# WeiZhang1988/YDORBSLAM

Hardware: AMD Instinct MI355X
Metric: ORB extract+match Mkeypoints/sec (higher is better)
Workload: dtype u8

## Files before the change

### ydorbslam_amd/csrc/extract_kernels.hip.h

```cpp
#pragma once
#include <hip/hip_runtime.h>
#include <stdint.h>

#include "quadtree_core.h"
#include "quadtree_flat.h"

#pragma clang fp contract(off)

namespace ydorb {

constexpr int kPad = 19;
constexpr int kBorder = 16;
constexpr int kMaxLevels = 8;
constexpr int kTileMax = 72;
#ifndef QT_THREADS
#define QT_THREADS 512
#endif
constexpr int kQtThreads = QT_THREADS;

struct LevelDev {
  int w, h, pitch;
  int padOff;
  int blurOff, blurPitch;
  int cellBegin, nCells;
  int quota;
  int candOff;
  int kpOff;
  int tabOff;
  int nodeTabOff;
  float scale;
  float size;
};
struct PlanDev {
  int nLevels, nCellsTotal, cellCap, sumQuota;
  int maxX[16];
  unsigned nodeTabFrameStride;
  int blurTileBegin[kMaxLevels + 1];
  int borderBegin[kMaxLevels + 1];
  LevelDev lv[kMaxLevels];
};
#ifndef BLUR_TH
#define BLUR_TH 58
#endif
constexpr int kBlurTW = 64, kBlurTH = BLUR_TH;
struct CellDev {
  short level, x0, y0, x1, y1, pad0;
  int srcOff;
};

__device__ __forceinline__ int reflect101(int i, int n) {
  if (n == 1) return 0;
  while (i < 0 || i >= n) i = i < 0 ? -i : 2 * (n - 1) - i;
  return i;
}

typedef uint32_t __attribute__((aligned(1))) u32_unaligned;
typedef unsigned long long __attribute__((aligned(1))) u64_unaligned;

#ifndef PYR_ROWS
#define PYR_ROWS 8
#endif
constexpr int kPyrRows = PYR_ROWS;
__global__ __launch_bounds__(256) void k_pyr_level0(const uint8_t* __restrict__ img, int stride, size_t frameStride,
                                                    uint8_t* __restrict__ pyr, size_t pyrFrameStride, LevelDev L) {
  const int wx = blockIdx.x * 64 + (threadIdx.x & 63);
  const int yb = (blockIdx.y * 4 + __builtin_amdgcn_readfirstlane(threadIdx.x >> 6)) * kPyrRows;
  const int x0 = wx * 4 - kPad;
  if (x0 + 3 < 0 || x0 >= L.w) return;
  const uint8_t* src = img + (size_t)blockIdx.z * frameStride;
  uint8_t* dst = pyr + (size_t)blockIdx.z * pyrFrameStride + L.padOff + (size_t)kPad * L.pitch + wx * 4;
  const int xa = L.w >= 4 ? min(max(x0, 0), L.w - 4) : 0, sh = 8 * (x0 - xa);
  uint32_t v[kPyrRows];
#pragma unroll
  for (int r = 0; r < kPyrRows; r++) {
    const uint8_t* row = src + (size_t)min(yb + r, L.h - 1) * stride;
    if (L.w >= 4) {
      v[r] = *reinterpret_cast<const u32_unaligned*>(row + xa);
    } else {
      v[r] = 0;
      for (int b = 0; b < L.w; b++) v[r] |= (uint32_t)row[b] << (8 * b);
    }
    v[r] = sh < 0 ? v[r] << (-sh) : v[r] >> sh;
  }
#pragma unroll
  for (int r = 0; r < kPyrRows; r++)
    if (yb + r < L.h) *reinterpret_cast<uint32_t*>(dst + (size_t)(yb + r) * L.pitch) = v[r];
}

__global__ __launch_bounds__(256) void k_pyr_resize(uint8_t* __restrict__ pyr, size_t pyrFrameStride, LevelDev Lp, LevelDev L,
                                                    double scaleX, const short* __restrict__ alpha,
                                                    const int* __restrict__ yofs, const short* __restrict__ beta) {
  const int wx = blockIdx.x * 64 + (threadIdx.x & 63);
  const int yb = (blockIdx.y * 4 + __builtin_amdgcn_readfirstlane(threadIdx.x >> 6)) * kPyrRows;
  const int x0 = wx * 4 - kPad;
  if (x0 + 3 < 0 || x0 >= L.w) return;
  uint8_t* frame = pyr + (size_t)blockIdx.z * pyrFrameStride;
  const uint8_t* S = frame + Lp.padOff + (size_t)kPad * Lp.pitch + kPad;
  uint8_t* dst = frame + L.padOff + (size_t)kPad * L.pitch + wx * 4;
  int sx[4], sx1[4], a0[4], a1[4];
#pragma unroll
  for (int b = 0; b < 4; b++) {
    const int dx = min(max(x0 + b, 0), L.w - 1);
    const float fx = (float)__dsub_rn(__dmul_rn((double)dx + 0.5, scaleX), 0.5);
    sx[b] = min(max((int)floorf(fx), 0), Lp.w - 1);
    a0[b] = alpha[2 * dx]; a1[b] = alpha[2 * dx + 1];
    sx1[b] = min(sx[b] + 1, Lp.w - 1);
  }
  const bool fast = sx[3] - sx[0] <= 6;
  const uint8_t *r0p[kPyrRows], *r1p[kPyrRows];
  int b0[kPyrRows], b1[kPyrRows];
#pragma unroll
  for (int r = 0; r < kPyrRows; r++) {
    const int dy = min(yb + r, L.h - 1);
    const int sy = yofs[dy];
    b0[r] = beta[2 * dy]; b1[r] = beta[2 * dy + 1];
    r0p[r] = S + (size_t)min(max(sy, 0), Lp.h - 1) * Lp.pitch;
    r1p[r] = S + (size_t)min(max(sy + 1, 0), Lp.h - 1) * Lp.pitch;
  }
  uint32_t v[kPyrRows];
  if (fast) {
    typedef unsigned short u16x2 __attribute__((ext_vector_type(2)));
    uint32_t sel[4];
    u16x2 ab[4];
#pragma unroll
    for (int b = 0; b < 4; b++) {
      const uint32_t off = (uint32_t)(sx[b] - sx[0]);
      sel[b] = off | 0x0c000c00u | ((off + 1) << 16);
      ab[b] = u16x2{(unsigned short)a0[b], (unsigned short)a1[b]};
    }
    unsigned long long w0[kPyrRows], w1[kPyrRows];
#pragma unroll
    for (int r = 0; r < kPyrRows; r++) {
      w0[r] = *reinterpret_cast<const u64_unaligned*>(r0p[r] + sx[0]);
      w1[r] = *reinterpret_cast<const u64_unaligned*>(r1p[r] + sx[0]);
    }
#pragma unroll
    for (int r = 0; r < kPyrRows; r++) {
      v[r] = 0;
#pragma unroll
      for (int b = 0; b < 4; b++) {
        const uint32_t p0 = __builtin_amdgcn_perm((uint32_t)(w0[r] >> 32), (uint32_t)w0[r], sel[b]);
        const uint32_t p1 = __builtin_amdgcn_perm((uint32_t)(w1[r] >> 32), (uint32_t)w1[r], sel[b]);
        const int h0 = (int)__builtin_amdgcn_udot2(__builtin_bit_cast(u16x2, p0), ab[b], 0u, false);
        const int h1 = (int)__builtin_amdgcn_udot2(__builtin_bit_cast(u16x2, p1), ab[b], 0u, false);
        const int o = (((b0[r] * (h0 >> 4)) >> 16) + ((b1[r] * (h1 >> 4)) >> 16) + 2) >> 2;
        v[r] |= (uint32_t)(o & 0xFF) << (8 * b);
      }
    }
  } else {
#pragma unroll
    for (int r = 0; r < kPyrRows; r++) {
      v[r] = 0;
#pragma unroll
      for (int b = 0; b < 4; b++) {
        const int h0 = r0p[r][sx[b]] * a0[b] + r0p[r][sx1[b]] * a1[b];
        const int h1 = r1p[r][sx[b]] * a0[b] + r1p[r][sx1[b]] * a1[b];
        const int o = (((b0[r] * (h0 >> 4)) >> 16) + ((b1[r] * (h1 >> 4)) >> 16) + 2) >> 2;
        v[r] |= (uint32_t)(o & 0xFF) << (8 * b);
      }
    }
  }
#pragma unroll
  for (int r = 0; r < kPyrRows; r++)
    if (yb + r < L.h) *reinterpret_cast<uint32_t*>(dst + (size_t)(yb + r) * L.pitch) = v[r];
}

struct PyrPadEntry { uint32_t laneA4, laneB4, selM, selF; };
struct PyrColEntry { uint32_t sel[4]; uint32_t ab[4]; };
constexpr uint32_t kPermIdentity = 0x03020100u;
#ifndef PYR_ROWS_F
#define PYR_ROWS_F 8
#endif
constexpr int kPyrRowsF = PYR_ROWS_F;

__device__ __forceinline__ uint32_t pyr_finish_dword(uint32_t v, const PyrPadEntry& pe) {
  const uint32_t A = (uint32_t)__builtin_amdgcn_ds_bpermute((int)pe.laneA4, (int)v);
  const uint32_t B = (uint32_t)__builtin_amdgcn_ds_bpermute((int)pe.laneB4, (int)v);
  const uint32_t M = __builtin_amdgcn_perm(A, B, pe.selM);
  return __builtin_amdgcn_perm(M, v, pe.selF);
}
__device__ __forceinline__ void pyr_store_rows(uint8_t* dst, int pitch, int y, int h, uint32_t v) {
  if (y >= h) return;
  *reinterpret_cast<uint32_t*>(dst + (ptrdiff_t)y * pitch) = v;
  if (y >= 1 && y <= kPad) *reinterpret_cast<uint32_t*>(dst - (ptrdiff_t)y * pitch) = v;
  if (y >= h - 1 - kPad && y <= h - 2) *reinterpret_cast<uint32_t*>(dst + (ptrdiff_t)(2 * (h - 1) - y) * pitch) = v;
}

__global__ __launch_bounds__(256) void k_pyr_level0_f(const uint8_t* __restrict__ img, int stride, size_t frameStride,
                                                      uint8_t* __restrict__ pyr, size_t pyrFrameStride, LevelDev L,
                                                      const PyrPadEntry* __restrict__ padTab, int shift) {
  const int wx = blockIdx.x * 64 + (threadIdx.x & 63) - shift;
  const int yb = (blockIdx.y * 4 + __builtin_amdgcn_readfirstlane(threadIdx.x >> 6)) * kPyrRowsF;
  const int nd = (L.w + 2 * kPad + 3) >> 2;
  if (wx < 0 || wx >= nd) return;
  const int x0 = wx * 4 - kPad;
  const uint8_t* src = img + (size_t)blockIdx.z * frameStride;
  uint8_t* dst = pyr + (size_t)blockIdx.z * pyrFrameStride + L.padOff + (size_t)kPad * L.pitch + wx * 4;
// ... 794 lines not shown
#pragma unroll
      for (int jj = 0; jj < 4; jj++) { key[jj] = (int)(st[4 * g + jj] & 0xFFFu); slot[jj] = qf_off(Pn) + (key[jj] >> (2 * (D - Pn))); }
      for (int d = Pn - 1; d >= 1; d--) {
        const int off = qf_off(d), sh = 2 * (D - d);
#pragma unroll
        for (int jj = 0; jj < 4; jj++) {
          const int sl = off + (key[jj] >> sh);
          if (hist[sl] == 1) slot[jj] = sl;
        }
      }
#pragma unroll
      for (int jj = 0; jj < 4; jj++) st[4 * g + jj] = (st[4 * g + jj] & 0xFFFF0000u) | (uint32_t)slot[jj];
    }
  }
  if (!pairs) {
    const int TQ = ((1 << (2 * Pn)) - 1) / 3;
    const int per = (TQ + NT - 1) / NT;
    constexpr int MAXQ = ((1 << (2 * D)) - 1) / 3 / NT + 1;
    uint2 qv[MAXQ];
    int qslot[MAXQ];
    unsigned flags = 0, cntF = 0;
#pragma unroll
    for (int t = 0; t < MAXQ; t++) {
      qslot[t] = -1; qv[t] = make_uint2(0, 0);
      const int q = tid * per + t;
      if (t < per && q < TQ) {
        int d = Pn, start = 0;
        while (q >= start + (1 << (2 * (d - 1)))) { start += 1 << (2 * (d - 1)); d--; }
        const int pq = q - start;
        const int bq = pq ^ (int)(qt_flat_mask(d) >> 2);
        qslot[t] = qf_off(d) + 4 * bq;
        qv[t] = *reinterpret_cast<const QT_LDS uint2*>(hist + qslot[t]);
        const unsigned c[4] = {qv[t].x & 0xFFFFu, qv[t].x >> 16, qv[t].y & 0xFFFFu, qv[t].y >> 16};
        const unsigned sum = c[0] + c[1] + c[2] + c[3];
#pragma unroll
        for (int e = 0; e < 4; e++) {
          const unsigned cn = c[3 - e];
          const bool fl = sum >= 2 && (d == Pn ? cn >= 1 : cn == 1);
          flags |= (unsigned)fl << (4 * t + e);
          cntF += fl;
        }
      }
    }
    unsigned total;
    unsigned pos = block_scan_excl(cntF, &total);
    if ((int)total != K) { give_up(); return; }
#pragma unroll
    for (int t = 0; t < MAXQ; t++) {
      if (qslot[t] >= 0) {
        const unsigned c[4] = {qv[t].x & 0xFFFFu, qv[t].x >> 16, qv[t].y & 0xFFFFu, qv[t].y >> 16};
        unsigned o[4];
#pragma unroll
        for (int e = 0; e < 4; e++) {
          const unsigned cn = c[3 - e];
          unsigned v = 0x7FFFu;
          if ((flags >> (4 * t + e)) & 1u) {
            if ((int)pos < nOut) {
              v = pos | (cn > 16 ? 0x8000u : 0u);
              if (cn > 16) nodeBig[pos] = 1;
            }
            pos++;
          }
          o[3 - e] = v;
        }
        *reinterpret_cast<QT_LDS uint2*>(hist + qslot[t]) = make_uint2(o[0] | (o[1] << 16), o[2] | (o[3] << 16));
      }
    }
  }
  __syncthreads();

#pragma unroll
  for (int g = 0; g < ITEMS / 4; g++) {
    if (4 * g * NT < n) {
      unsigned pv[4];
#pragma unroll
      for (int jj = 0; jj < 4; jj++) pv[jj] = pairs ? st[4 * g + jj] & 0x7FFFu : hist[st[4 * g + jj] & 0xFFFFu] & 0x7FFFu;
#pragma unroll
      for (int jj = 0; jj < 4; jj++) {
        const int i = (4 * g + jj) * NT + tid;
        const bool ok = i < n && (int)pv[jj] < nOut;
        const unsigned k = ok ? pv[jj] : (unsigned)(quotaMax + 1);
        const uint32_t rs = st[4 * g + jj] & 0xFFFF0000u;
        __hip_atomic_fetch_max(nodeLo + k, ok ? rs | (0xFFFFu - (uint32_t)i) : 0u, __ATOMIC_RELAXED, __HIP_MEMORY_SCOPE_WORKGROUP);
        __hip_atomic_fetch_max(nodeHi + k, ok ? rs | (uint32_t)i : 0u, __ATOMIC_RELAXED, __HIP_MEMORY_SCOPE_WORKGROUP);
        st[4 * g + jj] = rs | (ok ? k : 0xFFFFu);
      }
    }
  }
  __syncthreads();
  for (int k = tid; k < nOut; k += NT) {
    const unsigned iLo = 0xFFFFu - (nodeLo[k] & 0xFFFFu), iHi = nodeHi[k] & 0xFFFFu;
    if (iLo == iHi || !nodeBig[k]) {
      outKp[k] = fetch((int)iLo);
    } else {
      const int s = atomicAdd(&sTieN, 1);
      if (s < kQfMaxTied) { sTieNode[s] = k; nodeBig[k] = (uint8_t)(2 + s); }
    }
  }
  __syncthreads();
  const int nTied = sTieN;
  if (nTied > kQfMaxTied) { give_up(); return; }
  if (nTied > 0) {
    const int slotCap = kQfTieCap / nTied;
    QT_LDS uint32_t* tKey = (QT_LDS uint32_t*)smem;
    QT_LDS uint32_t* tVal = tKey + kQfTieCap;
#pragma unroll
    for (int j = 0; j < ITEMS; j++) {
      if (j * NT < n) {
        const unsigned k = st[j] & 0xFFFFu;
        if (k != 0xFFFFu) {
          const unsigned tb = nodeBig[k];
          if (tb >= 2) {
            const int s = (int)tb - 2, idx = atomicAdd(&sTieCnt[s], 1);
            if (idx < slotCap) { tKey[s * slotCap + idx] = (uint32_t)(j * NT + tid); tVal[s * slotCap + idx] = st[j] >> 16; }
            else sFlag = 1;
          }
        }
      }
    }
    __syncthreads();
    if (sFlag) { give_up(); return; }
    for (int s = 0; s < nTied; s++) {
      const int m = sTieCnt[s];
      constexpr int MAXM = (kQfTieCap + NT - 1) / NT;
      int rk[MAXM];
      uint32_t oi[MAXM], rr[MAXM];
#pragma unroll
      for (int t = 0; t < MAXM; t++) {
        rk[t] = -1; oi[t] = 0; rr[t] = 0;
        const int e = tid + NT * t;
        if (e < m) {
          oi[t] = tKey[s * slotCap + e];
          rr[t] = tVal[s * slotCap + e];
          int r = 0;
          for (int u = 0; u < m; u++) r += tKey[s * slotCap + u] < oi[t];
          rk[t] = r;
        }
      }
      __syncthreads();
#pragma unroll
      for (int t = 0; t < MAXM; t++)
        if (rk[t] >= 0) { tKey[s * slotCap + rk[t]] = (rr[t] << 16) | (uint32_t)rk[t]; tVal[s * slotCap + rk[t]] = oi[t]; }
      __syncthreads();
    }
    if (tid < nTied) {
      const int m = sTieCnt[tid];
      const int best = qt_sort_front(tKey + tid * slotCap, m);
      outKp[sTieNode[tid]] = fetch((int)tVal[tid * slotCap + best]);
    }
  }
  if (tid == 0) { needPass[unit] = 0; lvlCount[unit] = nOut; }
}

__global__ __launch_bounds__(256) void k_blur(const uint8_t* __restrict__ pyr, size_t pyrFrameStride, uint8_t* __restrict__ blur,
                                              size_t blurFrameStride, PlanDev P) {
  constexpr int TW = kBlurTW, TH = kBlurTH, SH = TH + 6, SWW = 18;
  __shared__ uint32_t src[SH * SWW];
  __shared__ __align__(16) uint32_t hb[(SH / 2) * TW];
  int f = blockIdx.y, tileId = blockIdx.x;
  if ((f | 7) < (int)gridDim.y) {
    tileId = (f & 7) * (gridDim.x >> 3) + (blockIdx.x >> 3);
    f = (f & ~7) | (blockIdx.x & 7);
  }
  if (tileId >= P.blurTileBegin[P.nLevels]) return;
  int level = 0;
#pragma unroll
  for (int l = 1; l < kMaxLevels; l++)
    if (l < P.nLevels && tileId >= P.blurTileBegin[l]) level = l;
  tileId -= P.blurTileBegin[level];
  const LevelDev L = P.lv[level];
  const int tilesX = (L.w + TW - 1) / TW;
  const int ty = tileId / tilesX, tx = tileId - ty * tilesX;
  const int x0 = tx * TW, y0 = ty * TH;
  const uint8_t* padded = pyr + (size_t)f * pyrFrameStride + L.padOff;
  {
    const int r0 = threadIdx.x / SWW, wd = threadIdx.x - r0 * SWW;
    const int pcol = x0 + 16 + 4 * wd;
    const bool colOk = pcol < L.pitch;
    if (r0 < 14)
#pragma unroll
      for (int r = r0; r < SH; r += 14) {
        const int prow = min(y0 + r + kPad - 3, L.h + 2 * kPad - 1);
        src[r * SWW + wd] = colOk ? *reinterpret_cast<const uint32_t*>(padded + (size_t)prow * L.pitch + pcol) : 0u;
      }
  }
  __syncthreads();
  for (int task = threadIdx.x; task < (SH / 2) * (TW / 4); task += 256) {
    const int rp = task >> 4, g = task & 15;
    uint32_t o[2][4];
#pragma unroll
    for (int h = 0; h < 2; h++) {
      const int r = 2 * rp + h;
      const uint32_t w0 = src[r * SWW + g], w1 = src[r * SWW + g + 1], w2 = src[r * SWW + g + 2];
#pragma unroll
      for (int k = 0; k < 4; k++) {
        const uint32_t lo4 = k ? __builtin_amdgcn_alignbyte(w1, w0, k) : w0, hi4 = k ? __builtin_amdgcn_alignbyte(w2, w1, k) : w1;
        o[h][k] = __builtin_amdgcn_udot4(hi4, 0x00122230u, __builtin_amdgcn_udot4(lo4, 0x38302212u, 0u, false), false);
      }
    }
    *reinterpret_cast<uint4*>(&hb[rp * TW + g * 4]) =
        make_uint4(o[0][0] | (o[1][0] << 16), o[0][1] | (o[1][1] << 16), o[0][2] | (o[1][2] << 16), o[0][3] | (o[1][3] << 16));
  }
  __syncthreads();
  const int c4 = (threadIdx.x & 15) * 4;
#pragma unroll
  for (int r = threadIdx.x >> 4; r < TH; r += 16) {
    const int gy = y0 + r;
    if (!(gy < L.h && x0 + c4 < L.blurPitch)) continue;
    typedef unsigned short u16x2 __attribute__((ext_vector_type(2)));
    const bool odd = r & 1;
    const u16x2 k0 = odd ? u16x2{0, 18} : u16x2{18, 34}, k1 = odd ? u16x2{34, 48} : u16x2{48, 56};
    const u16x2 k2 = odd ? u16x2{56, 48} : u16x2{48, 34}, k3 = odd ? u16x2{34, 18} : u16x2{18, 0};
    const uint32_t* hp = &hb[(r >> 1) * TW + c4];
    const uint4 p0 = *reinterpret_cast<const uint4*>(hp), p1 = *reinterpret_cast<const uint4*>(hp + TW);
    const uint4 p2 = *reinterpret_cast<const uint4*>(hp + 2 * TW), p3 = *reinterpret_cast<const uint4*>(hp + 3 * TW);
    const uint32_t q0[4] = {p0.x, p0.y, p0.z, p0.w}, q1[4] = {p1.x, p1.y, p1.z, p1.w}, q2[4] = {p2.x, p2.y, p2.z, p2.w}, q3[4] = {p3.x, p3.y, p3.z, p3.w};
    uint32_t acc[4];
#pragma unroll
    for (int k = 0; k < 4; k++) {
      acc[k] = __builtin_amdgcn_udot2(__builtin_bit_cast(u16x2, q0[k]), k0, 32768u, false);
      acc[k] = __builtin_amdgcn_udot2(__builtin_bit_cast(u16x2, q1[k]), k1, acc[k], false);
      acc[k] = __builtin_amdgcn_udot2(__builtin_bit_cast(u16x2, q2[k]), k2, acc[k], false);
      acc[k] = __builtin_amdgcn_udot2(__builtin_bit_cast(u16x2, q3[k]), k3, acc[k], false);
    }
    const uint32_t out = (acc[0] >> 16) | ((acc[1] >> 16) << 8) | ((acc[2] >> 16) << 16) | ((acc[3] >> 16) << 24);
    *reinterpret_cast<uint32_t*>(blur + (size_t)f * blurFrameStride + L.blurOff + (size_t)gy * L.blurPitch + x0 + c4) = out;
  }
}

__device__ __forceinline__ float fast_atan2_deg(float y, float x) {
  const float p1 = 0.9997878412794807f * (float)(180 / 3.14159265358979323846);
  const float p3 = -0.3258083974640975f * (float)(180 / 3.14159265358979323846);
  const float p5 = 0.1555786518463281f * (float)(180 / 3.14159265358979323846);
  const float p7 = -0.04432655554792128f * (float)(180 / 3.14159265358979323846);
  const float eps = (float)2.2204460492503131e-16;
  const float ax = fabsf(x), ay = fabsf(y);
  float a, c, c2;
  if (ax >= ay) {
    c = __fdiv_rn(ay, __fadd_rn(ax, eps));
    c2 = __fmul_rn(c, c);
    a = __fmul_rn(__fadd_rn(__fmul_rn(__fadd_rn(__fmul_rn(__fadd_rn(__fmul_rn(p7, c2), p5), c2), p3), c2), p1), c);
  } else {
    c = __fdiv_rn(ax, __fadd_rn(ay, eps));
    c2 = __fmul_rn(c, c);
    a = __fsub_rn(90.f, __fmul_rn(__fadd_rn(__fmul_rn(__fadd_rn(__fmul_rn(__fadd_rn(__fmul_rn(p7, c2), p5), c2), p3), c2), p1), c));
  }
  if (x < 0) a = __fsub_rn(180.f, a);
  if (y < 0) a = __fsub_rn(360.f, a);
  return a;
}

__device__ __forceinline__ void sincos_det(float xf, float* sinOut, float* cosOut) {
  const double x = (double)xf;
  const double n = rint(__dmul_rn(x, 6.36619772367581382433e-01));
  const double r = __dsub_rn(__dsub_rn(x, __dmul_rn(n, 1.57079632673412561417e+00)), __dmul_rn(n, 6.07710050650619224932e-11));
  const double z = __dmul_rn(r, r);
  double p = __dmul_rn(z, 1.58969099521155010221e-10);
  p = __dadd_rn(p, -2.50507602534068634195e-08); p = __dmul_rn(p, z);
  p = __dadd_rn(p, 2.75573137070700676789e-06);  p = __dmul_rn(p, z);
  p = __dadd_rn(p, -1.98412698298579493134e-04); p = __dmul_rn(p, z);
  p = __dadd_rn(p, 8.33333333332248946124e-03);  p = __dmul_rn(p, z);
  p = __dadd_rn(p, -1.66666666666666324348e-01); p = __dmul_rn(p, z);
  p = __dmul_rn(p, r); p = __dadd_rn(p, r);
  double q = __dmul_rn(z, -1.13596475577881948265e-11);
  q = __dadd_rn(q, 2.08757232129817482790e-09);  q = __dmul_rn(q, z);
  q = __dadd_rn(q, -2.75573143513906633035e-07); q = __dmul_rn(q, z);
  q = __dadd_rn(q, 2.48015872894767294178e-05);  q = __dmul_rn(q, z);
  q = __dadd_rn(q, -1.38888888888741095749e-03); q = __dmul_rn(q, z);
  q = __dadd_rn(q, 4.16666666666666019037e-02);  q = __dmul_rn(q, z);
  q = __dmul_rn(q, z);
  double h = __dmul_rn(z, 0.5);
  h = __dsub_rn(h, q);
  h = __dsub_rn(1.0, h);
  const int quad = ((int)n) & 3;
  const double sv = quad == 0 ? p : quad == 1 ? h : quad == 2 ? -p : -h;
  const double cv = quad == 0 ? h : quad == 1 ? -p : quad == 2 ? -h : p;
  *sinOut = (float)sv;
  *cosOut = (float)cv;
}

__device__ __align__(16) const float kPatternDev[1024] = {
#include "orb_pattern_data.inc"
};

struct YdKeyPointDev { float x, y, size, angle, response; int octave, class_id; };

__global__ __launch_bounds__(256) void k_orient_describe(const uint8_t* __restrict__ pyr, size_t pyrFrameStride,
                                                         const uint8_t* __restrict__ blur, size_t blurFrameStride, PlanDev P,
                                                         const uint32_t* __restrict__ lvlKp, const int* __restrict__ lvlCount,
                                                         YdKeyPointDev* __restrict__ kps, uint8_t* __restrict__ desc, int cap,
                                                         int* __restrict__ nOut, float* __restrict__ lvlAngle) {
  const int lane = threadIdx.x & 63;
  int bx = blockIdx.x, f = blockIdx.y;
  if ((f | 7) < (int)gridDim.y) {
    bx = (f & 7) * (gridDim.x >> 3) + (blockIdx.x >> 3);
    f = (f & ~7) | (blockIdx.x & 7);
  }
  const int slot = bx * 4 + __builtin_amdgcn_readfirstlane(threadIdx.x >> 6);
  if (slot >= P.sumQuota) return;
  float4 pat[4];
#pragma unroll
  for (int t = 0; t < 4; t++) pat[t] = reinterpret_cast<const float4*>(kPatternDev)[t * 64 + lane];
  int level = 0;
#pragma unroll
  for (int l = 1; l < kMaxLevels; l++)
    if (l < P.nLevels && slot >= P.lv[l].kpOff) level = l;
  const uint32_t pk = __builtin_amdgcn_readfirstlane(lvlKp[(size_t)f * P.sumQuota + slot]);
  int before = 0, tot = 0, mine = 0;
#pragma unroll
  for (int l = 0; l < kMaxLevels; l++) {
    const int c = l < P.nLevels ? lvlCount[f * kMaxLevels + l] : 0;
    if (l < level) before += c;
    if (l == level) mine = c;
    tot += c;
  }
  if (slot == 0 && lane == 0) nOut[f] = min(tot, cap);
  const LevelDev L = P.lv[level];
  const int k = slot - L.kpOff;
  if (k >= mine) return;
  const int outIdx = before + k;
  if (outIdx >= cap) return;
  const int kx = qt_x(pk) + kBorder, ky = qt_y(pk) + kBorder;
  const uint8_t* roi = pyr + (size_t)f * pyrFrameStride + L.padOff + (size_t)kPad * L.pitch + kPad;
  const uint8_t* org = roi + (ptrdiff_t)(ky - 15) * L.pitch + (kx - 32);
  const int u = lane - 32;
  unsigned narrow = 0;
#pragma unroll
  for (int v = 1; v <= 15; v++) narrow |= (unsigned)(P.maxX[v] == 0) << v;
  int m10 = 0, m01 = 0;
  if (u >= -15 && u <= 15) m10 = u * org[(unsigned)(15 * L.pitch + lane)];
  if (lane >= 1 && lane <= 15 && ((narrow >> lane) & 1u)) {
    const int pos = org[(unsigned)((15 + lane) * L.pitch + 32)], neg = org[(unsigned)((15 - lane) * L.pitch + 32)];
    m01 = lane * (pos - neg);
  }
#pragma unroll
  for (int v = 1; v <= 15; v++) {
    const int d = P.maxX[v];
    if (d > 0 && u >= -d && u <= d) {
      const int pos = org[(unsigned)((15 + v) * L.pitch + lane)], neg = org[(unsigned)((15 - v) * L.pitch + lane)];
      m01 += v * (pos - neg);
      m10 += u * (pos + neg);
    }
  }
#pragma unroll
  for (int o = 32; o >= 1; o >>= 1) {
    m10 += __shfl_xor(m10, o, 64);
    m01 += __shfl_xor(m01, o, 64);
  }
  const float angle = fast_atan2_deg((float)m01, (float)m10);
  const float rad = __fmul_rn(angle, (float)(3.14159265358979323846 / 180.0));
  float sinB, cosA;
  sincos_det(rad, &sinB, &cosA);
  constexpr int kBias = 24;
  const uint8_t* bl = blur + (size_t)f * blurFrameStride + L.blurOff + (ptrdiff_t)(ky - kBias) * L.blurPitch + (kx - kBias);
  unsigned long long words[4];
#pragma unroll
  for (int t = 0; t < 4; t++) {
    const float4 pt = pat[t];
    const int r0 = __float2int_rn(__fadd_rn(__fmul_rn(pt.x, sinB), __fmul_rn(pt.y, cosA)));
    const int c0 = __float2int_rn(__fsub_rn(__fmul_rn(pt.x, cosA), __fmul_rn(pt.y, sinB)));
    const int r1 = __float2int_rn(__fadd_rn(__fmul_rn(pt.z, sinB), __fmul_rn(pt.w, cosA)));
    const int c1 = __float2int_rn(__fsub_rn(__fmul_rn(pt.z, cosA), __fmul_rn(pt.w, sinB)));
    const int t0 = bl[(unsigned)((r0 + kBias) * L.blurPitch + c0 + kBias)], t1 = bl[(unsigned)((r1 + kBias) * L.blurPitch + c1 + kBias)];
    words[t] = __ballot(t0 < t1);
  }
  if (lane < 4) {
    unsigned long long w = lane == 0 ? words[0] : lane == 1 ? words[1] : lane == 2 ? words[2] : words[3];
    reinterpret_cast<unsigned long long*>(desc + ((size_t)f * cap + outIdx) * 32)[lane] = w;
  }
  if (lane == 0) {
    YdKeyPointDev kp;
    kp.x = (float)kx;
    kp.y = (float)ky;
    if (level) { kp.x = __fmul_rn(kp.x, L.scale); kp.y = __fmul_rn(kp.y, L.scale); }
    kp.size = L.size;
    kp.angle = angle;
    kp.response = (float)qt_r(pk);
    kp.octave = level;
    kp.class_id = -1;
// ... 158 lines not shown
```

### ydorbslam_amd/csrc/orb_extractor.hip

```cpp
#include <hip/hip_runtime.h>
#include <cstdlib>

#include <algorithm>
#include <cmath>
#include <cstdarg>
#include <cstdio>
#include <cstring>
#include <string>
#include <vector>

#include "../../include/ydorb/c_api.h"
#include "extract_kernels.hip.h"
#include "host_buffers.h"
#include "ydorb_host.h"

using namespace ydorb;

namespace {

inline int cvRoundF(float v) { return (int)lrintf(v); }
inline int cvFloorF(float v) { int i = (int)v; return i - (i > v); }
inline int alignUp(int v, int a) { return (v + a - 1) / a * a; }
inline size_t alignUpZ(size_t v, size_t a) { return (v + a - 1) / a * a; }

// ... 320 lines not shown
  HIPCHK(hipMalloc(&e->d_blur, P.blurFrameStride * B));
  HIPCHK(hipMalloc(&e->d_cellCount, sizeof(uint32_t) * D.nCellsTotal * B));
  HIPCHK(hipMalloc(&e->d_cellCand, sizeof(uint32_t) * (size_t)D.nCellsTotal * D.cellCap * B));
  HIPCHK(hipMalloc(&e->d_qtCand, sizeof(uint32_t) * 2 * P.qtFrameStride * B));
  HIPCHK(hipMalloc(&e->d_qtNode, sizeof(uint16_t) * 2 * P.qtFrameStride * B));
  if (D.nodeTabFrameStride) HIPCHK(hipMalloc(&e->d_nodeScratch, (size_t)D.nodeTabFrameStride * B));
  HIPCHK(hipMalloc(&e->d_needPass, (size_t)kMaxLevels * B));
  HIPCHK(hipMemsetAsync(e->d_needPass, 0, (size_t)kMaxLevels * B, e->stream));
  HIPCHK(hipMalloc(&e->d_passList, sizeof(int) * ((size_t)kMaxLevels * B + 1)));
  HIPCHK(hipMemsetAsync(e->d_passList, 0, sizeof(int), e->stream));

  HIPCHK(hipMalloc(&e->d_lvlKp, sizeof(uint32_t) * (size_t)D.sumQuota * B));
  HIPCHK(hipMalloc(&e->d_lvlAngle, sizeof(float) * (size_t)D.sumQuota * B));
  HIPCHK(hipMalloc(&e->d_lvlCount, sizeof(int) * kMaxLevels * B));
  HIPCHK(hipMalloc(&e->d_lvlMaxN, sizeof(int) * (kMaxLevels + 1)));
  HIPCHK(hipMemsetAsync(e->d_lvlMaxN, 0, sizeof(int) * (kMaxLevels + 1), e->stream));
  HIPCHK(hipHostMalloc(&e->h_lvlMaxN, sizeof(int) * (kMaxLevels + 1)));
  memset(e->h_lvlMaxN, 0, sizeof(int) * (kMaxLevels + 1));
  HIPCHK(hipMalloc(&e->d_status, sizeof(int)));
  HIPCHK(hipMalloc(&e->d_nOut, sizeof(int) * B));
  HIPCHK(hipMalloc(&e->d_cells, sizeof(CellDev) * std::max<size_t>(P.cells.size(), 1)));
  HIPCHK(hipMalloc(&e->d_tabInt, sizeof(int) * std::max<size_t>(P.tabInt.size(), 1)));
  HIPCHK(hipMalloc(&e->d_tabShort, sizeof(short) * std::max<size_t>(P.tabShort.size(), 1)));
  HIPCHK(hipMalloc(&e->d_kps, sizeof(YdKeyPointDev) * (size_t)D.sumQuota * B));
  HIPCHK(hipMalloc(&e->d_desc, (size_t)32 * D.sumQuota * B));
  HIPCHK(hipHostMalloc(&e->h_img, e->imgBytes * B));
  HIPCHK(hipHostMalloc(&e->h_kps, sizeof(YdKeyPoint) * (size_t)D.sumQuota * B));
  HIPCHK(hipHostMalloc(&e->h_desc, (size_t)32 * D.sumQuota * B));
  HIPCHK(hipHostMalloc(&e->h_nOut, sizeof(int) * B));
  HIPCHK(hipHostMalloc(&e->h_status, sizeof(int)));
  if (!P.cells.empty()) HIPCHK(hipMemcpyAsync(e->d_cells, P.cells.data(), sizeof(CellDev) * P.cells.size(), hipMemcpyHostToDevice, e->stream));
  if (!P.tabInt.empty()) HIPCHK(hipMemcpyAsync(e->d_tabInt, P.tabInt.data(), sizeof(int) * P.tabInt.size(), hipMemcpyHostToDevice, e->stream));
  if (!P.tabShort.empty()) HIPCHK(hipMemcpyAsync(e->d_tabShort, P.tabShort.data(), sizeof(short) * P.tabShort.size(), hipMemcpyHostToDevice, e->stream));
  HIPCHK(hipMalloc(&e->d_padTab, sizeof(PyrPadEntry) * std::max<size_t>(P.padTab.size(), 1)));
  HIPCHK(hipMalloc(&e->d_colTab, sizeof(PyrColEntry) * std::max<size_t>(P.colTab.size(), 1)));
  HIPCHK(hipMalloc(&e->d_rowTab, sizeof(int2) * std::max<size_t>(P.rowTab.size(), 1)));
  if (!P.padTab.empty()) HIPCHK(hipMemcpyAsync(e->d_padTab, P.padTab.data(), sizeof(PyrPadEntry) * P.padTab.size(), hipMemcpyHostToDevice, e->stream));
  if (!P.colTab.empty()) HIPCHK(hipMemcpyAsync(e->d_colTab, P.colTab.data(), sizeof(PyrColEntry) * P.colTab.size(), hipMemcpyHostToDevice, e->stream));
  if (!P.rowTab.empty()) HIPCHK(hipMemcpyAsync(e->d_rowTab, P.rowTab.data(), sizeof(int2) * P.rowTab.size(), hipMemcpyHostToDevice, e->stream));
  HIPCHK(hipMemsetAsync(e->d_status, 0, sizeof(int), e->stream));
  HIPCHK(hipStreamSynchronize(e->stream));
  if (std::max(P.qtLdsMax, P.qtPassLds) > 48 * 1024)
  {
    HIPCHK(hipFuncSetAttribute(reinterpret_cast<const void*>(k_quadtree), hipFuncAttributeMaxDynamicSharedMemorySize, (int)std::max(P.qtLdsMax, P.qtPassLds)));
    HIPCHK(hipFuncSetAttribute(reinterpret_cast<const void*>(k_quadtree_list), hipFuncAttributeMaxDynamicSharedMemorySize, (int)std::max(P.qtLdsMax, P.qtPassLds)));
  }
  {
    int qmax = 1, tabLen = 2;
    for (int l = 0; l < D.nLevels; l++) { qmax = std::max(qmax, D.lv[l].quota); tabLen = std::max(tabLen, std::max(D.lv[l].w - 2 * kBorder, 0) + std::max(D.lv[l].h - 2 * kBorder, 0) + 2); }
    const size_t ldsFast = std::min<size_t>(qt_fast_lds_bytes(qmax, tabLen), 150 * 1024);
    if (ldsFast > 48 * 1024) {
      HIPCHK(hipFuncSetAttribute(reinterpret_cast<const void*>(k_qt_fast<8>), hipFuncAttributeMaxDynamicSharedMemorySize, (int)ldsFast));
      HIPCHK(hipFuncSetAttribute(reinterpret_cast<const void*>(k_qt_fast<16>), hipFuncAttributeMaxDynamicSharedMemorySize, (int)ldsFast));
      HIPCHK(hipFuncSetAttribute(reinterpret_cast<const void*>(k_qt_fast<32>), hipFuncAttributeMaxDynamicSharedMemorySize, (int)ldsFast));
    }
  }
  e->planValid = true;
  return YDORB_OK;
}

void collectProfile(ydorb_extractor* e);

static void retuneQuadtree(ydorb_extractor* e) {
  HostPlan& P = e->plan;
  for (int l = 0; l < P.dev.nLevels; l++) {
    const int seen = e->h_lvlMaxN[l];
    if (seen > 0) P.qt[l].items = qfItemsFor((long)seen + seen / 8 + 32);
  }
}

int enqueue(ydorb_extractor* e, const uint8_t* d_img, int stride, size_t frameStride, int nFrames, YdKeyPointDev* d_kps,
            uint8_t* d_desc, int cap, int* d_nOut, hipStream_t s) {
  retuneQuadtree(e);
  const HostPlan& P = e->plan;
  const PlanDev& D = P.dev;
  const bool prof = e->profiling;
  if (prof) {
    if (e->profPending && hipEventQuery(e->ev[ST_COUNT]) == hipSuccess) collectProfile(e);
    e->profPending = false;
    HIPCHK(hipEventRecord(e->ev[0], s));
  }
  {
    const LevelDev& L0 = D.lv[0];
    auto fusedGrid = [&](const LevelDev& L, int shift) {
      return dim3((((L.w + 2 * kPad + 3) >> 2) + shift + 63) / 64, (L.h + 4 * kPyrRowsF - 1) / (4 * kPyrRowsF), nFrames);
    };
    if (P.fused[0].on) {
      hipLaunchKernelGGL(k_pyr_level0_f, fusedGrid(L0, P.fused[0].shift), dim3(256), 0, s, d_img, stride, frameStride, e->d_pyr, P.pyrFrameStride, L0,
                         e->d_padTab + P.fused[0].padOff, P.fused[0].shift);
    } else {
      dim3 g((L0.pitch / 4 + 63) / 64, (L0.h + 4 * kPyrRows - 1) / (4 * kPyrRows), nFrames);
      hipLaunchKernelGGL(k_pyr_level0, g, dim3(256), 0, s, d_img, stride, frameStride, e->d_pyr, P.pyrFrameStride, L0);
    }
    for (int l = 1; l < D.nLevels; l++) {
      const LevelDev& L = D.lv[l];
      const double scaleX = 1. / ((double)L.w / D.lv[l - 1].w);
      if (P.fused[l].on) {
        const HostPlan::FusedLevel& F = P.fused[l];
        hipLaunchKernelGGL(k_pyr_resize_f, fusedGrid(L, F.shift), dim3(256), 0, s, e->d_pyr, P.pyrFrameStride, D.lv[l - 1], L, scaleX,
                           e->d_colTab + F.colOff, e->d_padTab + F.padOff, e->d_rowTab + F.rowOff, F.shift);
      } else {
        dim3 gl((L.pitch / 4 + 63) / 64, (L.h + 4 * kPyrRows - 1) / (4 * kPyrRows), nFrames);
        hipLaunchKernelGGL(k_pyr_resize, gl, dim3(256), 0, s, e->d_pyr, P.pyrFrameStride, D.lv[l - 1], L, scaleX,
                           e->d_tabShort + P.tab[l].alpha, e->d_tabInt + P.tab[l].yofs, e->d_tabShort + P.tab[l].beta);
      }
    }
    if (D.borderBegin[D.nLevels] > 0)
      hipLaunchKernelGGL(k_pyr_borders, dim3(D.borderBegin[D.nLevels] / 256, nFrames), dim3(256), 0, s, e->d_pyr, P.pyrFrameStride, D);
  }
  if (prof) HIPCHK(hipEventRecord(e->ev[1], s));
  hipEvent_t fastEv[kMaxLevels]{};
  int grpFirst[kMaxLevels]{}, grpEnd[kMaxLevels]{}, nGroups = 0;
  {
    const int thr = std::min(std::max(e->cfg.ini_fast_thr, 0), 255);
    auto fastGeom = [&](int la, int lb, FastLds& fl, bool& narrow) -> size_t {
      int dim = 1;
      for (int l = la; l < lb; l++) dim = std::max(dim, P.levelCellDim[l]);
      const int maxT = dim + 6, maxB = dim;
      narrow = maxT <= 44;
      const int pitch = narrow ? 48 : 80;
      fl.tileBytes = alignUp((maxT + 3) * pitch, 16);
      fl.scoreBytes = alignUp((maxB + 2) * (maxB + 2) + 4, 16);
      fl.listBytes = alignUp(2 * maxB * maxB, 16);
      return (size_t)4 * (fl.tileBytes + fl.scoreBytes + fl.listBytes);
    };
    {
      FastLds flAll; bool nAll;
      const size_t dynAll = fastGeom(0, D.nLevels, flAll, nAll);
      if (dynAll > 48 * 1024) {
        HIPCHK(hipFuncSetAttribute(reinterpret_cast<const void*>(k_fast_cells<48>), hipFuncAttributeMaxDynamicSharedMemorySize, (int)dynAll));
        HIPCHK(hipFuncSetAttribute(reinterpret_cast<const void*>(k_fast_cells<80>), hipFuncAttributeMaxDynamicSharedMemorySize, (int)dynAll));
      }
    }
    int l0 = 0;
    for (int g = 0; g < e->fastGroups && l0 < D.nLevels; g++) {
      const int l1 = g == e->fastGroups - 1 ? D.nLevels : l0 + 1;
      const int c0 = D.lv[l0].cellBegin, c1 = D.lv[l1 - 1].cellBegin + D.lv[l1 - 1].nCells;
      if (c1 > c0 && D.nCellsTotal > 0) {
        FastLds fl; bool narrow;
        const size_t dyn = fastGeom(l0, l1, fl, narrow);
        const dim3 grid(((c1 - c0 + 3) / 4 + 7) / 8 * 8, nFrames);
        if (narrow) hipLaunchKernelGGL(k_fast_cells<48>, grid, dim3(256), dyn, s, e->d_pyr, P.pyrFrameStride, D, e->d_cells, c0, c1, thr, fl, e->d_cellCount, e->d_cellCand);
        else hipLaunchKernelGGL(k_fast_cells<80>, grid, dim3(256), dyn, s, e->d_pyr, P.pyrFrameStride, D, e->d_cells, c0, c1, thr, fl, e->d_cellCount, e->d_cellCand);
      }
      HIPCHK(hipEventRecord(e->evFast[l0], s));
      fastEv[l0] = e->evFast[l0];
      grpFirst[nGroups] = l0; grpEnd[nGroups] = l1; nGroups++;
      for (int l = l0 + 1; l < l1; l++) fastEv[l] = e->evFast[l0];
      l0 = l1;
    }
  }
  if (prof) HIPCHK(hipEventRecord(e->ev[2], s));
  HIPCHK(hipEventRecord(e->evFork, s));
  hipLaunchKernelGGL(k_blur, dim3((D.blurTileBegin[D.nLevels] + 7) / 8 * 8, nFrames), dim3(256), 0, s, e->d_pyr, P.pyrFrameStride, e->d_blur,
                     P.blurFrameStride, D);
  if (prof) HIPCHK(hipEventRecord(e->ev[3], s));
  bool anyFast = false;
  for (int g = 0; g < nGroups; g++) {
    const int l0 = grpFirst[g], l1 = grpEnd[g];
    const hipStream_t qs = e->qtInline ? s : e->qtStream[g % kMaxLevels];
    if (!e->qtInline) HIPCHK(hipStreamWaitEvent(qs, fastEv[l0] ? fastEv[l0] : e->evFork, 0));
    int items = 8, qmax = 1, tabLen = 2;
    for (int l = l0; l < l1; l++) {
      items = std::max(items, P.qt[l].items); qmax = std::max(qmax, D.lv[l].quota);
      tabLen = std::max(tabLen, std::max(D.lv[l].w - 2 * kBorder, 0) + std::max(D.lv[l].h - 2 * kBorder, 0) + 2);
    }
    const size_t lds = qt_fast_lds_bytes(qmax, tabLen);
    if (!e->forcePassQuadtree && lds <= 150 * 1024) {
      const dim3 grid(nFrames, l1 - l0);
#define YD_QT_FAST(IT) hipLaunchKernelGGL(k_qt_fast<IT>, grid, dim3(kQfThreads), lds, qs, D, e->d_cellCount, e->d_cellCand, l0, qmax, tabLen, e->d_lvlKp, \
                                          e->d_lvlCount, e->d_needPass, e->d_lvlMaxN, e->d_passList, e->d_passList + 1)
      if (items <= 8) YD_QT_FAST(8);
      else if (items <= 16) YD_QT_FAST(16);
      else YD_QT_FAST(32);
#undef YD_QT_FAST
      anyFast = true;
    } else {
      for (int l = l0; l < l1; l++) {
        const HostPlan::QtLevel& Q = P.qt[l];
        hipLaunchKernelGGL(k_quadtree, dim3(1, nFrames), dim3(kQtThreads), Q.lds, qs, D, e->d_cellCount, e->d_cellCand, e->d_qtCand, e->d_qtNode,
                           P.qtFrameStride, Q.nodeCap, Q.candCap, l, e->d_lvlKp, e->d_lvlCount, e->d_status, e->d_nodeScratch);
      }
    }
    if (!e->qtInline) HIPCHK(hipEventRecord(e->evJoin[g], qs));
  }
  if (!e->qtInline) for (int g = 0; g < nGroups; g++) HIPCHK(hipStreamWaitEvent(s, e->evJoin[g], 0));
  if (anyFast) {
    const int seen = e->h_lvlMaxN[kMaxLevels];
    const int listGrid = std::max(1, std::min({kQtPassWorkgroups, D.nLevels * nFrames, seen + seen / 4}));
    hipLaunchKernelGGL(k_quadtree_list, dim3(listGrid), dim3(kQtListThreads), P.qtPassLds, s, D, e->d_cellCount, e->d_cellCand,
                       e->d_qtCand, e->d_qtNode, P.qtFrameStride, -std::max(P.qtPassNodes, 1), e->d_lvlKp, e->d_lvlCount, e->d_status, e->d_passList,
                       e->d_passList + 1, e->d_nodeScratch, e->d_lvlMaxN + kMaxLevels);
    HIPCHK(hipMemsetAsync(e->d_passList, 0, sizeof(int), s));
  }
  if (prof) HIPCHK(hipEventRecord(e->ev[4], s));
  {
    const int kpw = e->descKpw;
    const dim3 gd(((D.sumQuota + 4 * kpw - 1) / (4 * kpw) + 7) / 8 * 8, nFrames);
#define YD_DESC(K) hipLaunchKernelGGL((k_orient_describe_n<K>), gd, dim3(256), 0, s, e->d_pyr, P.pyrFrameStride, e->d_blur, P.blurFrameStride, D, \
                                         e->d_lvlKp, e->d_lvlCount, d_kps, d_desc, cap, d_nOut, e->d_lvlAngle)
    if (kpw == 1)
      hipLaunchKernelGGL(k_orient_describe, gd, dim3(256), 0, s, e->d_pyr, P.pyrFrameStride, e->d_blur,
                         P.blurFrameStride, D, e->d_lvlKp, e->d_lvlCount, d_kps, d_desc, cap, d_nOut, e->d_lvlAngle);
    else if (kpw == 2) YD_DESC(2);
    else YD_DESC(4);
#undef YD_DESC
  }
  if (prof) { HIPCHK(hipEventRecord(e->ev[5], s)); e->profPending = true; }
  HIPCHK(hipMemcpyAsync(e->h_lvlMaxN, e->d_lvlMaxN, sizeof(int) * (kMaxLevels + 1), hipMemcpyDeviceToHost, s));
  HIPCHK(hipGetLastError());
  e->lastFrames = nFrames;
  e->lastStream = s;
  return YDORB_OK;
}

int checkStatus(ydorb_extractor* e) {
  if (*e->h_status == 1) { set_error("more than 65535 FAST candidates in one pyramid level"); return YDORB_ERR_CAPACITY; }
  if (*e->h_status == 3) { set_error("a pyramid level needs the pass quad-tree kernel (more candidates than LDS slots, or a very deep tree) but its quota is too large for that kernel's LDS node table"); return YDORB_ERR_CAPACITY; }
  if (*e->h_status) { set_error("quad-tree node table overflow (status %d)", *e->h_status); return YDORB_ERR_CAPACITY; }
  return YDORB_OK;
}

void collectProfile(ydorb_extractor* e) {
  if (!e->profiling || !e->profPending) return;
  e->profPending = false;
  for (int i = 0; i < ST_COUNT; i++) {
    float ms = 0;
    if (hipEventElapsedTime(&ms, e->ev[i], e->ev[i + 1]) == hipSuccess) e->stageMs[i] += ms;
  }
  e->stageCalls++;
}

}

int ydorb::extractor_pyramid_view(const ydorb_extractor* e, PyramidView* v) {
  if (!e || !v || !e->planValid || e->lastFrames < 1) { set_error("the extractor holds no pyramid (no call yet)"); return YDORB_ERR_INVALID_ARG; }
  v->device = e->cfg.device; v->nLevels = e->cfg.n_levels; v->frames = e->lastFrames; v->frameStride = (long long)e->plan.pyrFrameStride;
  v->stream = e->stream;
  for (int l = 0; l < e->cfg.n_levels; l++) {
    const LevelDev& L = e->plan.dev.lv[l];
    v->roi[l] = e->d_pyr + L.padOff + (size_t)kPad * L.pitch + kPad;
    v->w[l] = L.w; v->h[l] = L.h; v->pitch[l] = L.pitch;
    v->scale[l] = e->sf[l]; v->invScale[l] = e->isf[l];
    v->quota[l] = e->perLevel[l];
  }
  return YDORB_OK;
}

extern "C" {

int ydorb_extractor_create(const YdExtractorConfig* cfg, ydorb_extractor_t** out) {
  if (!cfg || !out) { set_error("null argument"); return YDORB_ERR_INVALID_ARG; }
  *out = nullptr;
  if (cfg->n_levels < 1 || cfg->n_levels > kMaxLevels || cfg->n_features < 1 || !(cfg->scale_factor > 1.0f)) {
    set_error("unsupported extractor config (n_levels 1..8, n_features >= 1, scale_factor > 1)");
    return YDORB_ERR_INVALID_ARG;
  }
  int rc = ydorb::require_device(cfg->device);
  if (rc) return rc;
  ydorb_extractor* e = new ydorb_extractor();
  e->cfg = *cfg;
  if (const char* v = getenv("YDORB_QT_PASS")) e->forcePassQuadtree = v[0] == '1';
  if (const char* v = getenv("YDORB_PYR_FUSED")) e->noFusedPads = v[0] == '0';
  e->descKpw = cfg->max_batch <= 8 ? 1 : 4;
  if (const char* v = getenv("YDORB_DESC_KPW")) e->descKpw = atoi(v) == 1 ? 1 : atoi(v) == 4 ? 4 : 2;
  e->cfg.min_fast_thr = cfg->ini_fast_thr;
  const int L = cfg->n_levels;
  const float s = cfg->scale_factor;
  int per = (int)round(cfg->n_features * (1 - 1.0 / s) / (1.0 - pow(1.0 / s, L)));
  int sum = 0;
  for (int i = 0; i < L; i++) {
    e->sf.push_back((float)pow(s, i));
    e->sf2.push_back((float)pow(s, 2 * i));
    e->isf.push_back((float)pow(s, -i));
    e->isf2.push_back((float)pow(s, -2 * i));
    if (i < L - 1) {
      e->perLevel.push_back(per);
      sum += per;
      per = (int)round((float)per / s);
    } else {
      e->perLevel.push_back(std::max(cfg->n_features - sum, 0));
    }
  }
  e->sumQuota = 0;
  for (int q : e->perLevel) e->sumQuota += q;
  {
    const int half = 15;
    std::vector<int> mx(half + 1, 0);
    const int maxY = (int)floor(half * sqrt(2.0) / 2.0 + 1.0), minY = (int)ceil(half * sqrt(2.0) / 2.0);
    for (int v = 0; v <= maxY; v++) mx.push_back((int)round(sqrt((double)half * half + (double)v * v)));
    for (int v = half, i = 0; v >= minY; v--) {
      while (mx[i] == mx[i + 1]) i++;
      mx[v] = i;
      i++;
    }
    for (int v = 0; v < 16; v++) e->maxX[v] = mx[v];
  }
  if (hipStreamCreateWithFlags(&e->stream, hipStreamNonBlocking) != hipSuccess) {
    set_error("hipStreamCreate failed");
    delete e;
    return YDORB_ERR_HIP;
  }
  for (auto& ev : e->ev) (void)hipEventCreate(&ev);
  (void)hipEventCreateWithFlags(&e->evFork, hipEventDisableTiming);
  for (int l = 0; l < kMaxLevels; l++) {
    const char* qtEnv = getenv("YDORB_QT_STREAMS");
    e->qtInline = (qtEnv && atoi(qtEnv) == 0) || (cfg->flags & YDORB_EXTRACTOR_SINGLE_STREAM);
// ... 266 lines not shown
```

Before: 181.8.

## Compute separable Gaussian blur with int8 MFMA matrix ops per single-wave tile

Rewrites the blur kernel so that one 64-thread wave per tile runs both the horizontal and vertical 7-tap passes as int8 32x32x32 MFMA products. The banded weight fragments are precomputed at compile time, and the horizontal result is split into high and low bytes so it fits the signed int8 inputs. The aim is to move the dot-product work from the VALU udot instructions onto the matrix cores and drop the shared-memory intermediate stage. In exchange it adds byte-split and sign-bias arithmetic, uses one wave per block, and stages output through an LDS tile before writing it out in 16-byte stores.

```diff
diff --git a/ydorbslam_amd/csrc/extract_kernels.hip.h b/ydorbslam_amd/csrc/extract_kernels.hip.h
--- a/ydorbslam_amd/csrc/extract_kernels.hip.h
+++ b/ydorbslam_amd/csrc/extract_kernels.hip.h
@@ -39,10 +39,7 @@
   int borderBegin[kMaxLevels + 1];
   LevelDev lv[kMaxLevels];
 };
-#ifndef BLUR_TH
-#define BLUR_TH 58
-#endif
-constexpr int kBlurTW = 64, kBlurTH = BLUR_TH;
+constexpr int kBlurTW = 64, kBlurTH = 58, kBlurThreads = 64;
 struct CellDev {
   short level, x0, y0, x1, y1, pad0;
   int srcOff;
@@ -1143,11 +1140,30 @@
   if (tid == 0) { needPass[unit] = 0; lvlCount[unit] = nOut; }
 }
 
-__global__ __launch_bounds__(256) void k_blur(const uint8_t* __restrict__ pyr, size_t pyrFrameStride, uint8_t* __restrict__ blur,
-                                              size_t blurFrameStride, PlanDev P) {
-  constexpr int TW = kBlurTW, TH = kBlurTH, SH = TH + 6, SWW = 18;
-  __shared__ uint32_t src[SH * SWW];
-  __shared__ __align__(16) uint32_t hb[(SH / 2) * TW];
+typedef int blur_i32x4 __attribute__((ext_vector_type(4)));
+typedef int blur_i32x16 __attribute__((ext_vector_type(16)));
+struct BlurFrags {
+  uint32_t th[2][64][4];
+  uint32_t tv[2][64][4];
+};
+constexpr uint32_t blur_weight(int d) { return d == 0 || d == 6 ? 18u : d == 1 || d == 5 ? 34u : d == 2 || d == 4 ? 48u : d == 3 ? 56u : 0u; }
+constexpr BlurFrags make_blur_frags() {
+  BlurFrags F{};
+  for (int q = 0; q < 2; q++)
+    for (int lane = 0; lane < 64; lane++)
+      for (int j = 0; j < 16; j++) {
+        const int n = lane & 31, h = lane >> 5;
+        F.th[q][lane][j >> 2] |= blur_weight(32 * q + 16 * h + j - n) << (8 * (j & 3));
+        F.tv[q][lane][j >> 2] |= blur_weight(32 * q + (j & 3) + 8 * (j >> 2) + 4 * h - n) << (8 * (j & 3));
+      }
+  return F;
+}
+static __device__ const BlurFrags kBlurFrags = make_blur_frags();
+
+__global__ __launch_bounds__(kBlurThreads, 2) void k_blur(const uint8_t* __restrict__ pyr, size_t pyrFrameStride, uint8_t* __restrict__ blur,
+                                                       size_t blurFrameStride, PlanDev P) {
+  constexpr int TW = kBlurTW, TH = kBlurTH;
+  static_assert(TW == 64 && TH > 32 && TH + 6 <= 64 && kBlurThreads == 64, "two 32-column strips and two 32-row blocks of source rows per wave");
   int f = blockIdx.y, tileId = blockIdx.x;
   if ((f | 7) < (int)gridDim.y) {
     tileId = (f & 7) * (gridDim.x >> 3) + (blockIdx.x >> 3);
@@ -1163,59 +1179,70 @@
   const int tilesX = (L.w + TW - 1) / TW;
   const int ty = tileId / tilesX, tx = tileId - ty * tilesX;
   const int x0 = tx * TW, y0 = ty * TH;
+  const int lane = threadIdx.x, n = lane & 31, h = lane >> 5;
+  const blur_i32x4 th0 = *reinterpret_cast<const blur_i32x4*>(kBlurFrags.th[0][lane]), th1 = *reinterpret_cast<const blur_i32x4*>(kBlurFrags.th[1][lane]);
+  const blur_i32x4 tv0 = *reinterpret_cast<const blur_i32x4*>(kBlurFrags.tv[0][lane]), tv1 = *reinterpret_cast<const blur_i32x4*>(kBlurFrags.tv[1][lane]);
   const uint8_t* padded = pyr + (size_t)f * pyrFrameStride + L.padOff;
-  {
-    const int r0 = threadIdx.x / SWW, wd = threadIdx.x - r0 * SWW;
-    const int pcol = x0 + 16 + 4 * wd;
-    const bool colOk = pcol < L.pitch;
-    if (r0 < 14)
-#pragma unroll
-      for (int r = r0; r < SH; r += 14) {
-        const int prow = min(y0 + r + kPad - 3, L.h + 2 * kPad - 1);
-        src[r * SWW + wd] = colOk ? *reinterpret_cast<const uint32_t*>(padded + (size_t)prow * L.pitch + pcol) : 0u;
-      }
+  const int pcol = x0 + 16 + 16 * h;
+  blur_i32x4 a[2][3];
+#pragma unroll
+  for (int mb = 0; mb < 2; mb++) {
+    const uint8_t* row = padded + (size_t)min(y0 + 32 * mb + n + kPad - 3, L.h + 2 * kPad - 1) * L.pitch + pcol;
+#pragma unroll
+    for (int s = 0; s < 3; s++) {
+      a[mb][s] = blur_i32x4{0, 0, 0, 0};
+      if (pcol + 32 * s < L.pitch && (s < 2 || h == 0)) a[mb][s] = *reinterpret_cast<const blur_i32x4*>(row + 32 * s);
+      a[mb][s] ^= (int)0x80808080;
+    }
+  }
+  constexpr int kRound = 128 * 256 * 256 + 128 * 256 + 32768;
+  blur_i32x16 round16;
+#pragma unroll
+  for (int i = 0; i < 16; i++) round16[i] = kRound;
+  asm volatile("" : "+v"(round16));
+  constexpr int TP = 80;
+  __shared__ __align__(16) uint8_t tile[64 * TP];
+  uint8_t* tl = tile + 4 * h * TP + n;
+#pragma unroll
+  for (int st = 0; st < 2; st++) {
+    blur_i32x4 hi[2], lo[2];
+#pragma unroll
+    for (int mb = 0; mb < 2; mb++) {
+      blur_i32x16 H = {};
+      H = __builtin_amdgcn_mfma_i32_32x32x32_i8(a[mb][st], th0, H, 0, 0, 0);
+      H = __builtin_amdgcn_mfma_i32_32x32x32_i8(a[mb][st + 1], th1, H, 0, 0, 0);
+#pragma unroll
+      for (int g = 0; g < 4; g++) {
+        const uint32_t p01 = __builtin_amdgcn_perm((uint32_t)H[4 * g + 1], (uint32_t)H[4 * g], 0x05040100u);
+        const uint32_t p23 = __builtin_amdgcn_perm((uint32_t)H[4 * g + 3], (uint32_t)H[4 * g + 2], 0x05040100u);
+        hi[mb][g] = (int)__builtin_amdgcn_perm(p23, p01, 0x07050301u);
+        lo[mb][g] = (int)(__builtin_amdgcn_perm(p23, p01, 0x06040200u) ^ 0x80808080u);
+      }
+    }
+#pragma unroll
+    for (int mb = 0; mb < 2; mb++) {
+      blur_i32x16 Shi = {}, Slo = round16;
+      if (mb == 0) {
+        Shi = __builtin_amdgcn_mfma_i32_32x32x32_i8(tv0, hi[0], Shi, 0, 0, 0);
+        Slo = __builtin_amdgcn_mfma_i32_32x32x32_i8(tv0, lo[0], Slo, 0, 0, 0);
+        Shi = __builtin_amdgcn_mfma_i32_32x32x32_i8(tv1, hi[1], Shi, 0, 0, 0);
+        Slo = __builtin_amdgcn_mfma_i32_32x32x32_i8(tv1, lo[1], Slo, 0, 0, 0);
+      } else {
+        Shi = __builtin_amdgcn_mfma_i32_32x32x32_i8(tv0, hi[1], Shi, 0, 0, 0);
+        Slo = __builtin_amdgcn_mfma_i32_32x32x32_i8(tv0, lo[1], Slo, 0, 0, 0);
+      }
+#pragma unroll
+      for (int i = 0; i < 16; i++)
+        tl[(32 * mb + (i & 3) + 8 * (i >> 2)) * TP + 32 * st] = (uint8_t)((uint32_t)(Shi[i] * 256 + Slo[i]) >> 16);
+    }
   }
   __syncthreads();
-  for (int task = threadIdx.x; task < (SH / 2) * (TW / 4); task += 256) {
-    const int rp = task >> 4, g = task & 15;
-    uint32_t o[2][4];
-#pragma unroll
-    for (int h = 0; h < 2; h++) {
-      const int r = 2 * rp + h;
-      const uint32_t w0 = src[r * SWW + g], w1 = src[r * SWW + g + 1], w2 = src[r * SWW + g + 2];
-#pragma unroll
-      for (int k = 0; k < 4; k++) {
-        const uint32_t lo4 = k ? __builtin_amdgcn_alignbyte(w1, w0, k) : w0, hi4 = k ? __builtin_amdgcn_alignbyte(w2, w1, k) : w1;
-        o[h][k] = __builtin_amdgcn_udot4(hi4, 0x00122230u, __builtin_amdgcn_udot4(lo4, 0x38302212u, 0u, false), false);
-      }
-    }
-    *reinterpret_cast<uint4*>(&hb[rp * TW + g * 4]) =
-        make_uint4(o[0][0] | (o[1][0] << 16), o[0][1] | (o[1][1] << 16), o[0][2] | (o[1][2] << 16), o[0][3] | (o[1][3] << 16));
-  }
-  __syncthreads();
-  const int c4 = (threadIdx.x & 15) * 4;
-#pragma unroll
-  for (int r = threadIdx.x >> 4; r < TH; r += 16) {
-    const int gy = y0 + r;
-    if (!(gy < L.h && x0 + c4 < L.blurPitch)) continue;
-    typedef unsigned short u16x2 __attribute__((ext_vector_type(2)));
-    const bool odd = r & 1;
-    const u16x2 k0 = odd ? u16x2{0, 18} : u16x2{18, 34}, k1 = odd ? u16x2{34, 48} : u16x2{48, 56};
-    const u16x2 k2 = odd ? u16x2{56, 48} : u16x2{48, 34}, k3 = odd ? u16x2{34, 18} : u16x2{18, 0};
-    const uint32_t* hp = &hb[(r >> 1) * TW + c4];
-    const uint4 p0 = *reinterpret_cast<const uint4*>(hp), p1 = *reinterpret_cast<const uint4*>(hp + TW);
-    const uint4 p2 = *reinterpret_cast<const uint4*>(hp + 2 * TW), p3 = *reinterpret_cast<const uint4*>(hp + 3 * TW);
-    const uint32_t q0[4] = {p0.x, p0.y, p0.z, p0.w}, q1[4] = {p1.x, p1.y, p1.z, p1.w}, q2[4] = {p2.x, p2.y, p2.z, p2.w}, q3[4] = {p3.x, p3.y, p3.z, p3.w};
-    uint32_t acc[4];
-#pragma unroll
-    for (int k = 0; k < 4; k++) {
-      acc[k] = __builtin_amdgcn_udot2(__builtin_bit_cast(u16x2, q0[k]), k0, 32768u, false);
-      acc[k] = __builtin_amdgcn_udot2(__builtin_bit_cast(u16x2, q1[k]), k1, acc[k], false);
-      acc[k] = __builtin_amdgcn_udot2(__builtin_bit_cast(u16x2, q2[k]), k2, acc[k], false);
-      acc[k] = __builtin_amdgcn_udot2(__builtin_bit_cast(u16x2, q3[k]), k3, acc[k], false);
-    }
-    const uint32_t out = (acc[0] >> 16) | ((acc[1] >> 16) << 8) | ((acc[2] >> 16) << 16) | ((acc[3] >> 16) << 24);
-    *reinterpret_cast<uint32_t*>(blur + (size_t)f * blurFrameStride + L.blurOff + (size_t)gy * L.blurPitch + x0 + c4) = out;
+  const int rows = min(TH, L.h - y0), c16 = 16 * (lane & 3);
+  uint8_t* out = blur + (size_t)f * blurFrameStride + L.blurOff + (size_t)y0 * L.blurPitch + x0 + c16;
+#pragma unroll
+  for (int q = 0; q < 4; q++) {
+    const int r = 16 * q + (lane >> 2);
+    if (r < rows) *reinterpret_cast<uint4*>(out + (size_t)r * L.blurPitch) = *reinterpret_cast<const uint4*>(tile + r * TP + c16);
   }
 }
 
diff --git a/ydorbslam_amd/csrc/orb_extractor.hip b/ydorbslam_amd/csrc/orb_extractor.hip
--- a/ydorbslam_amd/csrc/orb_extractor.hip
+++ b/ydorbslam_amd/csrc/orb_extractor.hip
@@ -496,7 +496,7 @@
   }
   if (prof) HIPCHK(hipEventRecord(e->ev[2], s));
   HIPCHK(hipEventRecord(e->evFork, s));
-  hipLaunchKernelGGL(k_blur, dim3((D.blurTileBegin[D.nLevels] + 7) / 8 * 8, nFrames), dim3(256), 0, s, e->d_pyr, P.pyrFrameStride, e->d_blur,
+  hipLaunchKernelGGL(k_blur, dim3((D.blurTileBegin[D.nLevels] + 7) / 8 * 8, nFrames), dim3(kBlurThreads), 0, s, e->d_pyr, P.pyrFrameStride, e->d_blur,
                      P.blurFrameStride, D);
   if (prof) HIPCHK(hipEventRecord(e->ev[3], s));
   bool anyFast = false;
```

Measured after the change: 181.7. About the same (-0.0%).
